# mingdeyu/DGP

Measured on AMD Instinct MI355X. Metric: SI iterations/sec (train) + predict pts/sec, 2-layer DGP n=2000 d=5, higher is better.
Workload: dtype f64; 1 GPU; configs[1]: 2-layer DGP, d=5 in / 1 out, n=2000, Matern-2.5, 5+1 GP nodes, train(ess_burn=10): one step = imputer.sample() + the M-step = one iteration of dgp.train (dgp.py:1364-1412); the same rate over a train(N=100) call is in `sustained`

## Files before the change

### dgp_amd/_lib.py

```python
import ctypes as C
import os

_HERE = os.path.dirname(os.path.abspath(__file__))
LIB_PATH = os.environ.get('DGPAMD_LIB') or os.path.join(_HERE, 'libdgp_amd.so')

OK, NOT_PD, BAD_ARG, HIP_ERROR = 0, 1, 2, 3
SEXP, MATERN25 = 0, 1
MAXD, MAXB = 64, 64
KIND = {'sexp': SEXP, 'matern2.5': MATERN25}

if not os.path.exists(LIB_PATH):
    raise ImportError(
        'dgp_amd: %s not found -- build it with `python -c "import __graft_entry__ as g; g.build()"` '
        '(or `make -C dgp_amd/csrc`).  dgp_amd has no CPU fallback.' % LIB_PATH)

lib = C.CDLL(LIB_PATH)

_p = C.c_void_p
_i = C.c_int
_l = C.c_int64
_d = C.c_double
_z = C.c_size_t

class Node(C.Structure):
# ... 29 lines not shown
    'dgpamd_set_linkgp_direct': (_i, [_p, _i]),
    'dgpamd_set_potrf_mode': (_i, [_p, _i]),
    'dgpamd_debug_trace': (_i, [_p, _p]),
    'dgpamd_debug_tasklog': (_i, [_p, _p, C.c_longlong]),
    'dgpamd_debug_mega_table': (_i, [_p, _l, _i, _i, _p, _l]),
    'dgpamd_prof_enable': (_i, [_p, _i]),
    'dgpamd_prof_event_overhead_us': (_i, [_p, C.POINTER(_d)]),
    'dgpamd_prof_collect': (_i, [_p, C.POINTER(_l), C.POINTER(_d), C.POINTER(_d)]),
    'dgpamd_kmatrix': (_i, [_p, _i, _l, _p, _l, _l, _p, _i, _p, _i, _p, _i, _d, _p, _p, _l, _l, _i, _p, _l, _l, _i, _i]),
    'dgpamd_potrf_workspace': (_z, [_l, _i]),
    'dgpamd_potrf': (_i, [_p, _l, _p, _l, _i, _p, _p, _p]),
    'dgpamd_aug_quad': (_i, [_p, _l, _p, _l, _i, _i, _p]),
    'dgpamd_loglik_finish': (_i, [_p, _l, _p, _l, _i, _p, _d, _p]),
    'dgpamd_loglik': (_i, [_p, _i, _l, _p, _l, _l, _p, _i, _p, _i, _p, _i, _d, _p, _d, _p, _p, _l, _i, _p, _p, _p]),
    'dgpamd_trmv_lower': (_i, [_p, _l, _p, _l, _p, _p, _p, _i]),
    'dgpamd_lik_workspace': (_z, [_i]),
    'dgpamd_lik_loglik': (_i, [_p, _p, _l, _i, _p, _l, _i, _p, _p]),
    'dgpamd_ess_propose': (_i, [_p, _l, _i, _p, _p, _p, _i, _p]),
    'dgpamd_potri': (_i, [_p, _l, _p, _p, _i, _p]),
    'dgpamd_potri_batched': (_i, [_p, _l, _p, _p, _l, _i, _i, _p]),
    'dgpamd_grad_workspace': (_z, [_l, _i]),
    'dgpamd_grad_reduce': (_i, [_p, _i, _l, _p, _l, _p, _i, _p, _i, _p, _i, _d, _p, _i, _p, _p, _p]),
    'dgpamd_ess_update': (_i, [_p, _l, _i, _p, _p, _p, _d, _d, _p, _p, _i, _i, _i, _p, _p, _p, _p, _p, _p]),
    'dgpamd_ess_queue_scratch': (_z, []),
    'dgpamd_ess_queue': (_i, [_p, _l, _i, _p, _p, _i, _p, _p, _i, _p, _p, _p, _i, _i, _i, _i, _i, _p, _p, _p, _p, _p]),
    'dgpamd_ess_queue_vwork': (_z, [_l, _i, _i]),
    'dgpamd_ess_queue_note_info': (_i, [_p, _p, _p, _i]),
    'dgpamd_llik_batch': (_i, [_p, _l, _i, _p, _p, _p, _p, _l, _p, _p, _p, _p, _l]),
    'dgpamd_llik_batch_launch': (_i, [_p, _l, _i, _p, _p, _p, _p, _l, _p, _p, _p, _l]),
    'dgpamd_llik_batch_wait': (_i, [_p, _p]),
# ... 60 lines not shown
```

### dgp_amd/csrc/chol.hip

```cpp
#include "common.hpp"
#include "tile.hpp"
#include "diagfac.hpp"

__device__ __forceinline__ void diag_logdet(DiagShared &sh, int ncol, int k, int b, int bad, double *logdet, int32_t *info) {
    const int tid = threadIdx.x;
    if (tid < 64) {
        const double pv = sh.piv[tid];
        double v = (tid < ncol && pv > 0.0) ? log(pv) : 0.0;
#pragma unroll
        for (int off = 32; off > 0; off >>= 1) v += __shfl_down(v, off, 64);
        if (tid == 0) {
            const double ld0 = k == 0 ? 0.0 : __hip_atomic_load(logdet + b, __ATOMIC_RELAXED, __HIP_MEMORY_SCOPE_AGENT);
            __hip_atomic_store(logdet + b, ld0 + v, __ATOMIC_RELAXED, __HIP_MEMORY_SCOPE_AGENT);
            int inf = k == 0 ? 0 : __hip_atomic_load(info + b, __ATOMIC_RELAXED, __HIP_MEMORY_SCOPE_AGENT);
            if (bad && inf == 0) inf = k * 64 + bad;
            __hip_atomic_store(info + b, inf, __ATOMIC_RELAXED, __HIP_MEMORY_SCOPE_AGENT);
        }
    }
}

enum { G_TRTRI1 = 2, G_TRTRI2 = 3, G_LAUUM = 4 };

struct GemmArgs {
    double *A;
// ... 1153 lines not shown
    const double *z;
    double *out;
    double sscale[DGPAMD_MAXB];
};
__global__ __launch_bounds__(256) void trmv_lower_kernel(TrmvArgs a) {
    const int b = blockIdx.y, wave = threadIdx.x >> 6, lane = threadIdx.x & 63;
    const int64_t i = (int64_t)blockIdx.x * 4 + wave;
    if (i >= a.n) return;
    const double *row = a.L + (int64_t)b * a.stride_a + i * a.ld;
    const double *z = a.z + (int64_t)b * a.n;
    double s = 0.0;
    for (int64_t j = lane; j <= i; j += 64) s = fma(row[j], z[j], s);
#pragma unroll
    for (int off = 32; off > 0; off >>= 1) s += __shfl_down(s, off, 64);
    if (lane == 0) a.out[(int64_t)b * a.n + i] = a.sscale[b] * s;
}

size_t potrf_ws_doubles(int64_t n, int batch) {
    int64_t nbk = padded_dim(n) / 64;
    return (size_t)batch * nbk * 4096 + 2 * DGPAMD_MAXB;
}

static size_t mega_sync_bytes(int64_t nbk, int batch);
static size_t mega_sync_offset(int64_t n, int batch) {
    const size_t b = potrf_ws_doubles(n, batch) * sizeof(double) + 3 * DGPAMD_MAXB * sizeof(int32_t);
    return (b + 127) / 128 * 128;
}
static size_t mega_piv_offset(int64_t n, int batch) {
    return mega_sync_offset(n, batch) + mega_sync_bytes(padded_dim(n) / 64, batch);
}
// ... 498 lines not shown
}

extern "C" int dgpamd_trmv_lower(dgpamd_ctx *ctx, int64_t n, const double *L, int64_t stride_a, const double *scale_h,
                                 const double *z, double *out, int batch) {
    if (!ctx) return DGPAMD_BAD_ARG;
    if (n <= 0 || !L || !z || !out || !scale_h) BAD_ARG(ctx, "null pointer or n <= 0");
    if (batch <= 0 || batch > DGPAMD_MAXB) BAD_ARG(ctx, "need 1 <= batch <= DGPAMD_MAXB");
    TrmvArgs a;
    a.L = L; a.ld = padded_dim(n); a.stride_a = stride_a; a.n = n; a.z = z; a.out = out;
    for (int b = 0; b < batch; ++b) a.sscale[b] = sqrt(scale_h[b]);
    hipLaunchKernelGGL(trmv_lower_kernel, dim3((unsigned)((n + 3) / 4), batch), dim3(256), 0, ctx->stream, a);
    LAUNCH_CHECK(ctx);
    return DGPAMD_OK;
}

static int potri_launches(dgpamd_ctx *ctx, int64_t n, double *A, double *Ainv, int64_t stride_a, int r, int batch,
                          void *work);

extern "C" int dgpamd_potri_batched(dgpamd_ctx *ctx, int64_t n, double *A, double *Ainv, int64_t stride_a, int r,
                                    int batch, void *work) {
    if (!ctx) return DGPAMD_BAD_ARG;
    if (n <= 0 || !A || !Ainv || !work || r < 0) BAD_ARG(ctx, "null pointer or n <= 0");
    if (batch <= 0 || batch > DGPAMD_MAXB) BAD_ARG(ctx, "need 1 <= batch <= DGPAMD_MAXB");
    const int64_t Np = padded_dim(n);
    if (n + r > Np) BAD_ARG(ctx, "too many right-hand sides");
    if (batch > 1 && stride_a < Np * Np) BAD_ARG(ctx, "stride_a < Np*Np");
    const std::array<uint64_t, 10> key = {2, (uint64_t)n, (uint64_t)r, (uint64_t)A, (uint64_t)Ainv, (uint64_t)work,
                                          (uint64_t)batch, (uint64_t)stride_a, 0, 0};
    return graph_run(ctx, key, [&]() { return potri_launches(ctx, n, A, Ainv, stride_a, r, batch, work); });
}
// ... 30 lines not shown
```

### dgp_amd/csrc/train.hip

```cpp
#include "common.hpp"
#include "wave.hpp"

#include <math.h>

struct ProposeArgs {
    const double *F, *NU;
    double *FP;
    int64_t count;
    double th[DGPAMD_MAXB];
};
__global__ __launch_bounds__(256) void ess_propose_kernel(ProposeArgs a) {
    const int b = blockIdx.y;
    const double c = cos(a.th[b]), s = sin(a.th[b]);
    for (int64_t i = (int64_t)blockIdx.x * 256 + threadIdx.x; i < a.count; i += (int64_t)gridDim.x * 256)
        a.FP[(int64_t)b * a.count + i] = a.F[i] * c + a.NU[i] * s;
}

extern "C" int dgpamd_ess_propose(dgpamd_ctx *ctx, int64_t n, int M, const double *F, const double *NU,
                                  const double *theta_h, int batch, double *FP) {
    if (!ctx) return DGPAMD_BAD_ARG;
    if (n <= 0 || M <= 0 || !F || !NU || !theta_h || !FP) BAD_ARG(ctx, "null pointer or empty block");
    if (batch <= 0 || batch > DGPAMD_MAXB) BAD_ARG(ctx, "need 1 <= batch <= DGPAMD_MAXB");
    ProposeArgs a;
    a.F = F; a.NU = NU; a.FP = FP; a.count = n * M;
// ... 641 lines not shown
                HIP_TRY(ctx, hipMemcpyAsync(F, FP + (int64_t)b * n * M, sizeof(double) * n * M, hipMemcpyDeviceToDevice,
                                            ctx->stream));
                return finish(0, llh[b], 0);
            }
        }
        used += nb - 1;
        proposals += nb;
        theta = th[nb - 1]; lo = blo[nb - 1]; hi = bhi[nb - 1];
        pending = true;
    }
}

enum { ES_THETA = 0, ES_LO, ES_HI, ES_PENDING, ES_CURSOR, ES_STATUS, ES_INFO, ES_LL, ES_LOGY, ES_PROPOSALS, ES_BATCHES,
       ES_UPDATES, ES_NWORDS = DGPAMD_ESS_STATE };
struct EssScratch {
    double th[DGPAMD_MAXB], lo[DGPAMD_MAXB], hi[DGPAMD_MAXB], cs[DGPAMD_MAXB], sn[DGPAMD_MAXB], ll[DGPAMD_MAXB], logdet[DGPAMD_MAXB];
    int32_t info[DGPAMD_MAXB], infomax[DGPAMD_MAXB];
    int32_t nb, done, acc, halt;
    double likpart[DGPAMD_MAXB * 32];
};
#define ESS_TWO_PI 6.283185307179586

__device__ void ess_prepare(double *st, const double *u, int nuni, int B, EssScratch *sc);
__global__ void ess_begin_kernel(double *st, const double *u, const double *logu, int nuni, EssScratch *sc, int upd, int B, int resume) {
    if (threadIdx.x) return;
    if (resume && upd == 0) {
        sc->done = 0;
        sc->halt = 0;
        ess_prepare(st, u, nuni, B, sc);
        return;
    }
    if (upd > 0 && !sc->done && st[ES_STATUS] == 0.0) st[ES_STATUS] = 3.0;
    sc->acc = -1;
    sc->nb = 0;
    if (st[ES_STATUS] != 0.0) { sc->done = 1; sc->halt = 1; return; }
    int cur = (int)st[ES_CURSOR];
    if (cur + 2 > nuni) { st[ES_STATUS] = 4.0; sc->done = 1; sc->halt = 1; return; }
    st[ES_LOGY] = st[ES_LL] + logu[cur];
    const double theta = ESS_TWO_PI * u[cur + 1];
    st[ES_THETA] = theta; st[ES_LO] = theta - ESS_TWO_PI; st[ES_HI] = theta; st[ES_PENDING] = 0.0;
    st[ES_CURSOR] = cur + 2;
    sc->done = 0;
    sc->halt = 0;
    ess_prepare(st, u, nuni, B, sc);
}
__device__ void ess_prepare(double *st, const double *u, int nuni, int B, EssScratch *sc) {
    sc->acc = -1;
    sc->nb = 0;
    if (sc->done) return;
    int cur = (int)st[ES_CURSOR];
    double theta = st[ES_THETA], lo = st[ES_LO], hi = st[ES_HI];
    if (st[ES_PENDING] != 0.0) {
        if (cur >= nuni) { st[ES_STATUS] = 1.0; sc->done = 1; return; }
        if (theta < 0.0) lo = theta; else hi = theta;
        theta = __dadd_rn(lo, __dmul_rn(hi - lo, u[cur++]));
        st[ES_THETA] = theta; st[ES_LO] = lo; st[ES_HI] = hi; st[ES_PENDING] = 0.0; st[ES_CURSOR] = cur;
    }
    int nb = 1;
    sc->th[0] = theta; sc->lo[0] = lo; sc->hi[0] = hi;
    while (nb < B && cur + nb - 1 < nuni) {
        if (theta < 0.0) lo = theta; else hi = theta;
        theta = __dadd_rn(lo, __dmul_rn(hi - lo, u[cur + nb - 1]));
        sc->th[nb] = theta; sc->lo[nb] = lo; sc->hi[nb] = hi;
        ++nb;
    }
    for (int b = nb; b < B; ++b) sc->th[b] = sc->th[nb - 1];
    for (int b = 0; b < B; ++b) { sc->cs[b] = cos(sc->th[b]); sc->sn[b] = sin(sc->th[b]); }
    sc->nb = nb;
}
__global__ void ess_prepare_kernel(double *st, const double *u, int nuni, int B, EssScratch *sc) {
    if (threadIdx.x) return;
    ess_prepare(st, u, nuni, B, sc);
}
__global__ __launch_bounds__(256) void ess_propose_dev_kernel(const double *F, const double *NU, double *FP, int64_t count,
                                                              const EssScratch *sc) {
    if (sc->done) return;
    const int b = blockIdx.y;
    const double c = sc->cs[b], s = sc->sn[b];
    for (int64_t i = (int64_t)blockIdx.x * 256 + threadIdx.x; i < count; i += (int64_t)gridDim.x * 256)
        FP[(int64_t)b * count + i] = F[i] * c + NU[i] * s;
}
__device__ void ess_decide(double *st, EssScratch *sc);
__global__ void ess_node_ll_kernel(const double *A, int64_t ld, int64_t stride_a, int64_t n, double scale, int B, int first,
                                   EssScratch *sc, const double *ld_ws, const int32_t *info_ws, const int32_t *status, double *st) {
    const int b = threadIdx.x;
    if (sc->done) return;
    if (b < B) {
        const double logdet = ld_ws ? __hip_atomic_load(ld_ws + b, __ATOMIC_RELAXED, __HIP_MEMORY_SCOPE_AGENT) : sc->logdet[b];
        const int32_t info = ld_ws ? ((status && __hip_atomic_load(status, __ATOMIC_RELAXED, __HIP_MEMORY_SCOPE_AGENT))
                                          ? -1 : __hip_atomic_load(info_ws + b, __ATOMIC_RELAXED, __HIP_MEMORY_SCOPE_AGENT))
                                   : sc->info[b];
        const double quad = -A[(int64_t)b * stride_a + n * ld + n];
        const double ll = -0.5 * ((double)n * log(scale) + logdet + quad / scale);
        sc->ll[b] = (first ? 0.0 : sc->ll[b]) + ll;
        sc->infomax[b] = first ? info : (sc->infomax[b] ? sc->infomax[b] : info);
    }
    if (st) {
        __threadfence_block();
        __syncthreads();
        if (b == 0) ess_decide(st, sc);
    }
}
__device__ void ess_decide(double *st, EssScratch *sc) {
    if (sc->done) return;
    const int nb = sc->nb;
    int cur = (int)st[ES_CURSOR];
    st[ES_BATCHES] += 1.0;
    for (int b = 0; b < nb; ++b) {
        if (sc->infomax[b] != 0) {
            st[ES_STATUS] = 2.0; st[ES_INFO] = sc->infomax[b]; st[ES_PROPOSALS] += b + 1; sc->done = 1;
            return;
        }
        if (sc->ll[b] > st[ES_LOGY]) {
            st[ES_CURSOR] = cur + b; st[ES_PROPOSALS] += b + 1;
            st[ES_THETA] = sc->th[b]; st[ES_LO] = sc->lo[b]; st[ES_HI] = sc->hi[b]; st[ES_PENDING] = 0.0;
            st[ES_LL] = sc->ll[b]; st[ES_UPDATES] += 1.0;
            sc->acc = b; sc->done = 1;
            return;
        }
    }
    st[ES_CURSOR] = cur + nb - 1; st[ES_PROPOSALS] += nb;
    st[ES_THETA] = sc->th[nb - 1]; st[ES_LO] = sc->lo[nb - 1]; st[ES_HI] = sc->hi[nb - 1]; st[ES_PENDING] = 1.0;
}
__global__ __launch_bounds__(256) void ess_accept_kernel(double *F, const double *FP, int64_t count, const EssScratch *sc) {
    const int acc = sc->acc;
    if (acc < 0) return;
    for (int64_t i = (int64_t)blockIdx.x * 256 + threadIdx.x; i < count; i += (int64_t)gridDim.x * 256)
        F[i] = FP[(int64_t)acc * count + i];
}
__global__ void ess_end_kernel(double *st, EssScratch *sc) {
    if (threadIdx.x) return;
    if (!sc->done && st[ES_STATUS] == 0.0) st[ES_STATUS] = 3.0;
    sc->acc = -1;
}
__global__ void ess_set_ll_kernel(double *st, const EssScratch *sc) {
    if (threadIdx.x) return;
    if (st[ES_STATUS] != 0.0) return;
    if (sc->infomax[0] != 0) { st[ES_STATUS] = 2.0; st[ES_INFO] = sc->infomax[0]; }
    st[ES_LL] = sc->ll[0];
}
__global__ void ess_note_info_kernel(double *st, const int32_t *info, int count) {
    if (threadIdx.x || st[ES_STATUS] != 0.0) return;
    for (int i = 0; i < count; ++i)
// ... 21 lines not shown
        const int64_t src = a.ord[i];
        a.out[(int64_t)b * total + e] = d < a.Dl ? a.X[(int64_t)b * a.stride_x + src * a.M + a.colmap[d]] : a.Xglob[src * a.Dg + (d - a.Dl)];
    }
}
__global__ void ess_vnode_ll_kernel(const double *o, double scale, int B, int first, EssScratch *sc, double *st) {
    const int b = threadIdx.x;
    if (sc->done) return;
    if (b < B) {
        const double ll = -0.5 * (o[2 * b + 1] + o[2 * b] / scale);
        sc->ll[b] = (first ? 0.0 : sc->ll[b]) + ll;
        if (first) sc->infomax[b] = 0;
    }
    if (st) {
        __threadfence_block();
        __syncthreads();
        if (b == 0) ess_decide(st, sc);
    }
}

#define LIK_CHUNKS 32
struct LikArgs {
    const double *X;
    int64_t stride_x;
    int M, kind, ncol, classes;
    int cols[DGPAMD_MAXD];
    const int64_t *rep;
    const double *y;
    int64_t nobs;
    double par;
    double *part;
    const int32_t *pred;
// ... 113 lines not shown
    for (int c = 0; c < LIK_CHUNKS; ++c) s += part[b * LIK_CHUNKS + c];
    out[b] = s;
}
__global__ void ess_liknode_ll_kernel(const double *part, int B, int first, EssScratch *sc, double *st) {
    const int b = threadIdx.x;
    if (sc->done) return;
    if (b < B) {
        double s = 0.0;
        for (int c = 0; c < LIK_CHUNKS; ++c) s += part[b * LIK_CHUNKS + c];
        sc->ll[b] = (first ? 0.0 : sc->ll[b]) + s;
        if (first) sc->infomax[b] = 0;
    }
    if (st) {
        __threadfence_block();
        __syncthreads();
        if (b == 0) ess_decide(st, sc);
    }
}
static int lik_launch(dgpamd_ctx *ctx, const dgpamd_node &nd, int64_t n, int M, const double *X, int64_t stride_x, int B, double *part) {
    if (nd.lik_kind < DGPAMD_LIK_POISSON || nd.lik_kind > DGPAMD_LIK_SOFTMAX) BAD_ARG(ctx, "unknown likelihood");
    if (!nd.y || nd.lik_nobs <= 0 || !nd.colmap || nd.Dl <= 0 || nd.Dl > DGPAMD_MAXD) BAD_ARG(ctx, "incomplete likelihood node");
    static const int need[] = {0, 1, 2, 2, 3, 1, 1, 0, 0};
    if (need[nd.lik_kind] && nd.Dl != need[nd.lik_kind]) BAD_ARG(ctx, "wrong number of latent columns for this likelihood");
    if (nd.lik_kind >= DGPAMD_LIK_ROBUSTMAX && (nd.lik_classes != nd.Dl || nd.Dl < 2)) BAD_ARG(ctx, "one latent column per class");
    if (!nd.lik_rep && nd.lik_nobs != n) BAD_ARG(ctx, "observations and latent rows differ without a replicate map");
    LikArgs a;
    a.X = X; a.stride_x = stride_x; a.M = M; a.kind = nd.lik_kind; a.ncol = nd.Dl; a.classes = nd.lik_classes;
    for (int d = 0; d < nd.Dl; ++d) {
        a.cols[d] = ((const int32_t *)nd.colmap)[d];
        if (a.cols[d] < 0 || a.cols[d] >= M) BAD_ARG(ctx, "latent column out of range");
    }
// ... 8 lines not shown
    int rc = lik_launch(ctx, *node, n, M, X, stride_x, batch, work);
    if (rc) return rc;
    hipLaunchKernelGGL(lik_sum_kernel, dim3(1), dim3(DGPAMD_MAXB), 0, ctx->stream, (const double *)work, batch, out);
    LAUNCH_CHECK(ctx);
    return DGPAMD_OK;
}
extern "C" size_t dgpamd_lik_workspace(int batch) { return (size_t)batch * LIK_CHUNKS * sizeof(double); }

extern "C" size_t dgpamd_ess_queue_scratch(void) { return (sizeof(EssScratch) + 15) / 16 * 16; }
extern "C" size_t dgpamd_ess_queue_vwork(int64_t n, int D, int batch) {
    return ((size_t)batch * n * (D + 2) + 2 * (size_t)batch + 2) * sizeof(double);
}

static int ess_queue_logliks(dgpamd_ctx *ctx, int64_t n, int M, const double *X, int64_t stride_x, int B, const dgpamd_node *nodes,
                             const double *scales_h, int nnodes, double *A, void *work, EssScratch *sc, double *st_decide, void *vwork,
                             int vbatch) {
    const int64_t Np = padded_dim(n);
    double *ws = (double *)work;
    for (int k = 0; k < nnodes; ++k) {
        const dgpamd_node &nd = nodes[k];
        if (nd.lik_kind) {
            int rc = lik_launch(ctx, nd, n, M, X, stride_x, B, sc->likpart);
            if (rc) return rc;
            hipLaunchKernelGGL(ess_liknode_ll_kernel, dim3(1), dim3(DGPAMD_MAXB), 0, ctx->stream, (const double *)sc->likpart, B,
                               k == 0 ? 1 : 0, sc, k == nnodes - 1 ? st_decide : nullptr);
            continue;
        }
        if (!(scales_h[k] > 0.0)) BAD_ARG(ctx, "scale must be positive");
        if (nd.vecch_nn) {
            const int D = nd.Dl + nd.Dg;
            if (!vwork || !nd.vecch_ord || !nd.vecch_nd || !nd.vecch_y || nd.vecch_m < 0) BAD_ARG(ctx, "incomplete Vecchia node");
// ... 21 lines not shown
            hipLaunchKernelGGL(ess_vnode_ll_kernel, dim3(1), dim3(DGPAMD_MAXB), 0, ctx->stream, (const double *)osum, scales_h[k], B,
                               k == 0 ? 1 : 0, sc, k == nnodes - 1 ? st_decide : nullptr);
            continue;
        }
        if (!A || !work) BAD_ARG(ctx, "dense nodes upstairs need A and work");
        KmatArgs a;
        int rc = build_kmat_args(ctx, a, nd.kind, n, X, M, stride_x, (const int32_t *)nd.colmap, nd.Dl, nd.Xglob, nd.Dg, nd.length,
                                 nd.nlen, nd.nugget, nd.W, A, Np, Np * Np, 0, nd.y, n, 0, 1, B);
        if (rc) return rc;
        potrf_sync_area(ctx, n, B, false, ws, &a.zero_ptr, &a.zero_words);
        rc = launch_kmatrix(ctx, a, B);
        if (rc) return rc;
        PotrfPost post;
        rc = run_potrf(ctx, n, A, Np * Np, B, sc->logdet, sc->info, ws, nullptr, nullptr, &post, a.zero_ptr != nullptr);
        if (rc) return rc;
        hipLaunchKernelGGL(ess_node_ll_kernel, dim3(1), dim3(DGPAMD_MAXB), 0, ctx->stream, (const double *)A, Np, Np * Np, n,
                           scales_h[k], B, k == 0 ? 1 : 0, sc, post.pending ? post.ld_ws : nullptr,
                           post.pending ? post.info_ws : nullptr, post.pending ? post.status : nullptr,
                           k == nnodes - 1 ? st_decide : nullptr);
    }
    LAUNCH_CHECK(ctx);
    return DGPAMD_OK;
}

extern "C" int dgpamd_ess_queue(dgpamd_ctx *ctx, int64_t n, int M, double *F, const double *NU, int nupd, const dgpamd_node *nodes,
                                const double *scales_h, int nnodes, double *state, const double *uniforms, const double *log_uniforms,
                                int nuni, int batch_first, int batch_next, int max_batches, int compute_ll0, double *FP, double *A,
                                void *work, void *scratch, void *vwork) {
    if (!ctx) return DGPAMD_BAD_ARG;
    if (n <= 0 || M <= 0 || nupd <= 0 || nnodes <= 0 || !F || !NU || !nodes || !scales_h || !state || !FP || !scratch)
        BAD_ARG(ctx, "null pointer or empty block");
    if (nuni < 0 || (nuni > 0 && (!uniforms || !log_uniforms))) BAD_ARG(ctx, "bad uniform stream");
    if (batch_first <= 0 || batch_first > DGPAMD_MAXB) BAD_ARG(ctx, "need 1 <= batch_first <= DGPAMD_MAXB");
    if (batch_next <= 0 || batch_next > batch_first) batch_next = batch_first;
    if (max_batches < 1) max_batches = 1;
    EssScratch *sc = reinterpret_cast<EssScratch *>(scratch);
    const int64_t count = n * (int64_t)M;
    int64_t blocks = (count + 255) / 256;
    if (blocks > 1024) blocks = 1024;
    int rc;
    HIP_TRY(ctx, hipMemsetAsync(sc, 0, sizeof(EssScratch), ctx->stream));
    const int resume = compute_ll0 == 2 ? 1 : 0;
    if (compute_ll0 == 1) {
        rc = ess_queue_logliks(ctx, n, M, F, 0, 1, nodes, scales_h, nnodes, A, work, sc, nullptr, vwork, batch_first);
        if (rc) return rc;
        hipLaunchKernelGGL(ess_set_ll_kernel, dim3(1), dim3(64), 0, ctx->stream, state, (const EssScratch *)sc);
    }
    for (int u = 0; u < nupd; ++u) {
        const double *NUu = NU + (int64_t)u * count;
        hipLaunchKernelGGL(ess_begin_kernel, dim3(1), dim3(64), 0, ctx->stream, state, uniforms, log_uniforms, nuni, sc, u, batch_first, resume);
        for (int j = 0; j < max_batches; ++j) {
            const int B = j == 0 ? batch_first : batch_next;
            if (j > 0) hipLaunchKernelGGL(ess_prepare_kernel, dim3(1), dim3(64), 0, ctx->stream, state, uniforms, nuni, B, sc);
            hipLaunchKernelGGL(ess_propose_dev_kernel, dim3((unsigned)blocks, B), dim3(256), 0, ctx->stream, (const double *)F, NUu, FP,
                               count, (const EssScratch *)sc);
            ctx->pred = &sc->done;
            rc = ess_queue_logliks(ctx, n, M, FP, count, B, nodes, scales_h, nnodes, A, work, sc, state, vwork, batch_first);
            ctx->pred = nullptr;
            if (rc) return rc;
            hipLaunchKernelGGL(ess_accept_kernel, dim3((unsigned)blocks), dim3(256), 0, ctx->stream, F, (const double *)FP, count,
                               (const EssScratch *)sc);
        }
        if (u == nupd - 1) hipLaunchKernelGGL(ess_end_kernel, dim3(1), dim3(64), 0, ctx->stream, state, sc);
    }
    LAUNCH_CHECK(ctx);
    return DGPAMD_OK;
}

extern "C" int dgpamd_ess_queue_note_info(dgpamd_ctx *ctx, double *state, const int32_t *info, int count) {
    if (!ctx) return DGPAMD_BAD_ARG;
    if (!state || !info || count <= 0) BAD_ARG(ctx, "bad arguments");
    hipLaunchKernelGGL(ess_note_info_kernel, dim3(1), dim3(64), 0, ctx->stream, state, info, count);
    LAUNCH_CHECK(ctx);
    return DGPAMD_OK;
}
```

### dgp_amd/imputation.py

```python
import os
import numpy as np
from numpy.linalg import LinAlgError
from .ops import raise_not_pd
from . import dist as ddist
import torch

from .ops import default_engine
from .kernel_class import TrackedInputs, bind_private, peek

TWO_PI = 2.0 * np.pi
_NO_UPLOAD_AHEAD = bool(__import__('os').environ.get('DGPAMD_NO_UPLOAD_AHEAD'))


class DrawStream:

    def __init__(self, seed=None, z=None, u=None):
        ss = seed if isinstance(seed, np.random.SeedSequence) else np.random.SeedSequence(seed)
        a, b = ss.spawn(2)
        self._gz, self._gu = np.random.default_rng(a), np.random.default_rng(b)
        self._z = None if z is None else [np.asarray(v, dtype=float) for v in z]
        self._ubuf = [] if u is None else [float(v) for v in u]
        self._injected_u = u is not None
        self._zbuf, self._zpos, self._thread = None, 0, None

# ... 666 lines not shown
        if self.draws._z is not None and len(self.all_layer) > 2:
            return None
        e = self.engine
        n, M = self.F[0].shape
        if M > 64:
            return None
        if all_vecch:
            Zd = self._normals_ahead(sweeps, M, n)
            xs = self._vecchia_draws(0, list(range(M)), Zd.permute(1, 0, 2).contiguous())
            if prefetch:
                self.draws.prefetch(sweeps * M * n, engine=e)
            return xs.permute(1, 2, 0).contiguous()
        buf = self._layer_factors(0, list(range(M)))
        Zd = self._normals_ahead(sweeps, M, n)
        scales = [float(nd.scale[0]) for nd in layer]
        out = e.empty(sweeps, M, n)
        for s_ in range(sweeps):
            e.trmv_lower(n, buf, scales, Zd[s_], batch=M, out=out[s_])
        if prefetch:
            self.draws.prefetch(sweeps * M * n, engine=e)
        return out.transpose(1, 2).contiguous()

    def _prior_draw(self, l, cols=None):
        e = self.engine
        layer = self.all_layer[l]
        n, M = self.F[l].shape
        Np = e.padded_dim(n)
        nu = e.zeros(n, M)
        cols = list(range(M)) if cols is None else list(cols)
        dense = [k for k in cols if not layer[k].vecch]
        Z = {k: self.draws.normal(n) for k in cols}
        if dense:
            buf = self._layer_factors(l, dense)
# ... 354 lines not shown
```

### dgp_amd/ops.py

```python
import ctypes as C

import numpy as np
import torch

import os

from . import _lib
from ._lib import lib, KIND

_NO_PINNED_UPLOAD = os.environ.get('DGPAMD_PINNED_UPLOAD') == '0'
_POISON_ALL = os.environ.get('DGPAMD_POISON_LDS') == '2'
_POISON_HBM = os.environ.get('DGPAMD_POISON_HBM') == '1'


class DgpAmdError(RuntimeError):
    pass


class HandoffError(DgpAmdError):
    """The one-launch factorisation gave up waiting for another workgroup (its workgroups were not co-resident: a device
    shared with another process, a debugger, a time-sliced partition).  Not a numerical failure; the per-block-step
    factorisation (Engine.set_potrf_mode(0)) has no such waits -- dgp.train retries the iteration once through it."""


# ... 234 lines not shown
        stride_loc = n * ldloc if Xloc.dim() == 3 else 0
        self._chk(self._enter() or lib.dgpamd_loglik(self.h, KIND[kind], n, _dp(Xloc), ldloc, stride_loc, cmp_, Dl, _dp(Xglob), Dg,
                                    _hp(length), len(length), float(nugget), _dp(W), float(scale), _dp(y), _dp(A),
                                    Np * Np, batch, _dp(ll), _dp(info), _dp(work)))
        return ll, info

    def trmv_lower(self, n, L, scale, z, batch=1, out=None, shared=False):
        Np = self.padded_dim(n)
        sc = _f64(scale)
        if len(sc) == 1 and batch > 1:
            sc = np.repeat(sc, batch)
        if out is None:
            out = self.empty(batch, n)
        self._chk(self._enter() or lib.dgpamd_trmv_lower(self.h, n, _dp(L), 0 if shared else Np * Np, _hp(sc), _dp(z), _dp(out),
                                                          batch))
        return out

    def ess_propose(self, F, NU, thetas, out=None):
        n, M = F.shape
        th = _f64(thetas)
        B = len(th)
        if out is None:
            out = self.empty(B, n, M)
        self._chk(self._enter() or lib.dgpamd_ess_propose(self.h, n, M, _dp(F), _dp(NU), _hp(th), B, _dp(out)))
        return out

    def potri(self, n, A, Ainv, r, work, batch=1):
        Np = self.padded_dim(n)
        self._chk(self._enter() or lib.dgpamd_potri_batched(self.h, n, _dp(A), _dp(Ainv), Np * Np if batch > 1 else 0, r, batch, _dp(work)))
        return Ainv
# ... 850 lines not shown
```

### include/dgp_amd.h

```cpp
#ifndef DGP_AMD_H
#define DGP_AMD_H

#include <stddef.h>
#include <stdint.h>

#ifdef __cplusplus
extern "C" {
#endif

#define DGPAMD_OK 0
#define DGPAMD_NOT_PD 1
#define DGPAMD_BAD_ARG 2
#define DGPAMD_HIP_ERROR 3

#define DGPAMD_SEXP 0
#define DGPAMD_MATERN25 1

#define DGPAMD_MAXD 64
#define DGPAMD_MAXB 64

typedef struct dgpamd_ctx dgpamd_ctx;

int dgpamd_create(int device, void *stream, dgpamd_ctx **out);
int dgpamd_destroy(dgpamd_ctx *ctx);
// ... 38 lines not shown

int dgpamd_loglik_finish(dgpamd_ctx *ctx, int64_t n, const double *A, int64_t stride_a, int batch, const double *logdet,
                         double scale, double *ll);

int dgpamd_gemv(dgpamd_ctx *ctx, int64_t rows, int64_t cols, const double *A, int64_t ld, const double *x, double *out);

int dgpamd_loglik(dgpamd_ctx *ctx, int kind, int64_t n,
                  const double *Xloc, int64_t ldloc, int64_t stride_loc, const int32_t *colmap_h, int Dl,
                  const double *Xglob, int Dg,
                  const double *length_h, int nlen, double nugget, const double *W, double scale,
                  const double *y, double *A, int64_t stride_a, int batch,
                  double *ll, int32_t *info, void *work);

int dgpamd_trmv_lower(dgpamd_ctx *ctx, int64_t n, const double *L, int64_t stride_a, const double *scale_h,
                      const double *z, double *out, int batch);

int dgpamd_ess_propose(dgpamd_ctx *ctx, int64_t n, int M, const double *F, const double *NU,
                       const double *theta_h, int batch, double *FP);

int dgpamd_potri(dgpamd_ctx *ctx, int64_t n, double *A, double *Ainv, int r, void *work);
int dgpamd_potrf_inv(dgpamd_ctx *ctx, int64_t n, double *A, double *T, double *S, int64_t stride_a, int batch,
                     double *logdet, int32_t *info, void *work);

int dgpamd_potri_batched(dgpamd_ctx *ctx, int64_t n, double *A, double *Ainv, int64_t stride_a, int r, int batch,
                         void *work);

typedef struct {
    int kind;
    int Dl, Dg, nlen;
    int nugget_est;
// ... 223 lines not shown
```

Measured before the change: 31.46 SI it/s.

## Fuse ESS begin/prepare into propose kernel and batch multi-column TRMV

The ESS begin and prepare single-thread kernels are folded into the proposal kernel: each workgroup recomputes its theta from a shared-memory window of uniforms, and the last workgroup, picked with an atomic ticket, writes the state back. For single-node layers, the node log-likelihood and accept/reject decision are folded into the accept kernel the same way. Separately, the per-sweep TRMV loop that draws prior samples is replaced by one kernel that handles many right-hand-side columns at once, reusing each loaded row of L. This cuts kernel launches and serial tiny kernels in the ESS loop, at the cost of redundant per-block computation, ticket-based cross-block coordination, and changed FMA rounding in theta updates.

```diff
diff --git a/dgp_amd/_lib.py b/dgp_amd/_lib.py
--- a/dgp_amd/_lib.py
+++ b/dgp_amd/_lib.py
@@ -67,6 +67,7 @@
     'dgpamd_loglik_finish': (_i, [_p, _l, _p, _l, _i, _p, _d, _p]),
     'dgpamd_loglik': (_i, [_p, _i, _l, _p, _l, _l, _p, _i, _p, _i, _p, _i, _d, _p, _d, _p, _p, _l, _i, _p, _p, _p]),
     'dgpamd_trmv_lower': (_i, [_p, _l, _p, _l, _p, _p, _p, _i]),
+    'dgpamd_trmv_lower_multi': (_i, [_p, _l, _p, _l, _p, _p, _p, _i, _i, _l]),
     'dgpamd_lik_workspace': (_z, [_i]),
     'dgpamd_lik_loglik': (_i, [_p, _p, _l, _i, _p, _l, _i, _p, _p]),
     'dgpamd_ess_propose': (_i, [_p, _l, _i, _p, _p, _p, _i, _p]),
diff --git a/dgp_amd/csrc/chol.hip b/dgp_amd/csrc/chol.hip
--- a/dgp_amd/csrc/chol.hip
+++ b/dgp_amd/csrc/chol.hip
@@ -1191,6 +1191,38 @@
 #pragma unroll
     for (int off = 32; off > 0; off >>= 1) s += __shfl_down(s, off, 64);
     if (lane == 0) a.out[(int64_t)b * a.n + i] = a.sscale[b] * s;
+}
+
+#define TRMV_COLS 12
+struct TrmvMultiArgs {
+    TrmvArgs t;
+    int64_t col_stride;
+    int ncols;
+};
+__global__ __launch_bounds__(256) void trmv_lower_multi_kernel(TrmvMultiArgs a) {
+    const int b = blockIdx.y, wave = threadIdx.x >> 6, lane = threadIdx.x & 63;
+    const int64_t i = (int64_t)blockIdx.x * 4 + wave;
+    if (i >= a.t.n) return;
+    const double *row = a.t.L + (int64_t)b * a.t.stride_a + i * a.t.ld;
+    for (int c0 = 0; c0 < a.ncols; c0 += TRMV_COLS) {
+        const int nc = a.ncols - c0 < TRMV_COLS ? a.ncols - c0 : TRMV_COLS;
+        const double *z = a.t.z + (int64_t)c0 * a.col_stride + (int64_t)b * a.t.n;
+        double s[TRMV_COLS];
+#pragma unroll
+        for (int c = 0; c < TRMV_COLS; ++c) s[c] = 0.0;
+        for (int64_t j = lane; j <= i; j += 64) {
+            const double l = row[j];
+#pragma unroll
+            for (int c = 0; c < TRMV_COLS; ++c)
+                if (c < nc) s[c] = fma(l, z[(int64_t)c * a.col_stride + j], s[c]);
+        }
+#pragma unroll
+        for (int c = 0; c < TRMV_COLS; ++c) {
+#pragma unroll
+            for (int off = 32; off > 0; off >>= 1) s[c] += __shfl_down(s[c], off, 64);
+            if (lane == 0 && c < nc) a.t.out[(int64_t)(c0 + c) * a.col_stride + (int64_t)b * a.t.n + i] = a.t.sscale[b] * s[c];
+        }
+    }
 }
 
 size_t potrf_ws_doubles(int64_t n, int batch) {
@@ -1719,6 +1751,22 @@
     return DGPAMD_OK;
 }
 
+extern "C" int dgpamd_trmv_lower_multi(dgpamd_ctx *ctx, int64_t n, const double *L, int64_t stride_a, const double *scale_h,
+                                       const double *z, double *out, int batch, int ncols, int64_t col_stride) {
+    if (!ctx) return DGPAMD_BAD_ARG;
+    if (n <= 0 || !L || !z || !out || !scale_h) BAD_ARG(ctx, "null pointer or n <= 0");
+    if (batch <= 0 || batch > DGPAMD_MAXB) BAD_ARG(ctx, "need 1 <= batch <= DGPAMD_MAXB");
+    if (ncols <= 0) BAD_ARG(ctx, "need ncols >= 1");
+    if (ncols > 1 && col_stride < (int64_t)batch * n) BAD_ARG(ctx, "col_stride < batch * n");
+    TrmvMultiArgs a;
+    a.t.L = L; a.t.ld = padded_dim(n); a.t.stride_a = stride_a; a.t.n = n; a.t.z = z; a.t.out = out;
+    for (int b = 0; b < batch; ++b) a.t.sscale[b] = sqrt(scale_h[b]);
+    a.col_stride = col_stride; a.ncols = ncols;
+    hipLaunchKernelGGL(trmv_lower_multi_kernel, dim3((unsigned)((n + 3) / 4), batch), dim3(256), 0, ctx->stream, a);
+    LAUNCH_CHECK(ctx);
+    return DGPAMD_OK;
+}
+
 static int potri_launches(dgpamd_ctx *ctx, int64_t n, double *A, double *Ainv, int64_t stride_a, int r, int batch,
                           void *work);
 
diff --git a/dgp_amd/csrc/train.hip b/dgp_amd/csrc/train.hip
--- a/dgp_amd/csrc/train.hip
+++ b/dgp_amd/csrc/train.hip
@@ -679,119 +679,228 @@
 enum { ES_THETA = 0, ES_LO, ES_HI, ES_PENDING, ES_CURSOR, ES_STATUS, ES_INFO, ES_LL, ES_LOGY, ES_PROPOSALS, ES_BATCHES,
        ES_UPDATES, ES_NWORDS = DGPAMD_ESS_STATE };
 struct EssScratch {
-    double th[DGPAMD_MAXB], lo[DGPAMD_MAXB], hi[DGPAMD_MAXB], cs[DGPAMD_MAXB], sn[DGPAMD_MAXB], ll[DGPAMD_MAXB], logdet[DGPAMD_MAXB];
+    double th[DGPAMD_MAXB], lo[DGPAMD_MAXB], hi[DGPAMD_MAXB], spare[2 * DGPAMD_MAXB], ll[DGPAMD_MAXB], logdet[DGPAMD_MAXB];
     int32_t info[DGPAMD_MAXB], infomax[DGPAMD_MAXB];
     int32_t nb, done, acc, halt;
+    int32_t ticket, fill_;
     double likpart[DGPAMD_MAXB * 32];
 };
 #define ESS_TWO_PI 6.283185307179586
 
-__device__ void ess_prepare(double *st, const double *u, int nuni, int B, EssScratch *sc);
-__global__ void ess_begin_kernel(double *st, const double *u, const double *logu, int nuni, EssScratch *sc, int upd, int B, int resume) {
-    if (threadIdx.x) return;
-    if (resume && upd == 0) {
-        sc->done = 0;
-        sc->halt = 0;
-        ess_prepare(st, u, nuni, B, sc);
-        return;
-    }
-    if (upd > 0 && !sc->done && st[ES_STATUS] == 0.0) st[ES_STATUS] = 3.0;
-    sc->acc = -1;
-    sc->nb = 0;
-    if (st[ES_STATUS] != 0.0) { sc->done = 1; sc->halt = 1; return; }
-    int cur = (int)st[ES_CURSOR];
-    if (cur + 2 > nuni) { st[ES_STATUS] = 4.0; sc->done = 1; sc->halt = 1; return; }
-    st[ES_LOGY] = st[ES_LL] + logu[cur];
-    const double theta = ESS_TWO_PI * u[cur + 1];
-    st[ES_THETA] = theta; st[ES_LO] = theta - ESS_TWO_PI; st[ES_HI] = theta; st[ES_PENDING] = 0.0;
-    st[ES_CURSOR] = cur + 2;
-    sc->done = 0;
-    sc->halt = 0;
-    ess_prepare(st, u, nuni, B, sc);
-}
-__device__ void ess_prepare(double *st, const double *u, int nuni, int B, EssScratch *sc) {
-    sc->acc = -1;
-    sc->nb = 0;
-    if (sc->done) return;
-    int cur = (int)st[ES_CURSOR];
-    double theta = st[ES_THETA], lo = st[ES_LO], hi = st[ES_HI];
-    if (st[ES_PENDING] != 0.0) {
-        if (cur >= nuni) { st[ES_STATUS] = 1.0; sc->done = 1; return; }
+__device__ __forceinline__ double ess_rounded(double x) {
+    asm volatile("" : "+v"(x));
+    return x;
+}
+#define ESS_UWIN (DGPAMD_MAXB + 4)
+struct EssUniforms {
+    const double *win;
+    int base;
+    __device__ __forceinline__ double operator()(int i) const { return win[i - base]; }
+};
+struct EssOpened {
+    int done;
+    double theta;
+};
+template <bool W>
+__device__ __forceinline__ EssOpened ess_open(double *st, const EssUniforms &u, const double *logu, int nuni, EssScratch *sc, int upd, int B,
+                                              int resume, int sel) {
+    int done = sc->done;
+    double status = st[ES_STATUS], curd = st[ES_CURSOR], theta = st[ES_THETA], lo = st[ES_LO], hi = st[ES_HI], pending = st[ES_PENDING];
+    EssOpened r;
+    r.theta = theta;
+    if (upd >= 0) {
+        if (resume && upd == 0) {
+            done = 0;
+            if (W) { sc->done = 0; sc->halt = 0; }
+        } else {
+            if (upd > 0 && !done && status == 0.0) {
+                status = 3.0;
+                if (W) st[ES_STATUS] = 3.0;
+            }
+            if (W) { sc->acc = -1; sc->nb = 0; }
+            const int cur = (int)curd;
+            if (status != 0.0 || cur + 2 > nuni) {
+                if (W) {
+                    if (status == 0.0) st[ES_STATUS] = 4.0;
+                    sc->done = 1;
+                    sc->halt = 1;
+                }
+                r.done = 1;
+                return r;
+            }
+            const double u1 = u(cur + 1);
+            theta = ess_rounded(ESS_TWO_PI * u1);
+            lo = fma(ESS_TWO_PI, u1, -ESS_TWO_PI);
+            hi = theta;
+            pending = 0.0;
+            curd = cur + 2;
+            done = 0;
+            if (W) {
+                st[ES_LOGY] = st[ES_LL] + logu[cur];
+                st[ES_THETA] = theta; st[ES_LO] = lo; st[ES_HI] = hi; st[ES_PENDING] = 0.0;
+                st[ES_CURSOR] = curd;
+                sc->done = 0;
+                sc->halt = 0;
+            }
+        }
+    }
+    if (W) { sc->acc = -1; sc->nb = 0; }
+    r.done = done;
+    if (done) return r;
+    int cur = (int)curd;
+    if (pending != 0.0) {
+        if (cur >= nuni) {
+            if (W) { st[ES_STATUS] = 1.0; sc->done = 1; }
+            r.done = 1;
+            return r;
+        }
         if (theta < 0.0) lo = theta; else hi = theta;
-        theta = __dadd_rn(lo, __dmul_rn(hi - lo, u[cur++]));
-        st[ES_THETA] = theta; st[ES_LO] = lo; st[ES_HI] = hi; st[ES_PENDING] = 0.0; st[ES_CURSOR] = cur;
+        theta = fma(hi - lo, u(cur), lo);
+        ++cur;
+        if (W) { st[ES_THETA] = theta; st[ES_LO] = lo; st[ES_HI] = hi; st[ES_PENDING] = 0.0; st[ES_CURSOR] = cur; }
     }
     int nb = 1;
-    sc->th[0] = theta; sc->lo[0] = lo; sc->hi[0] = hi;
+    if (W) { sc->th[0] = theta; sc->lo[0] = lo; sc->hi[0] = hi; }
+    r.theta = theta;
     while (nb < B && cur + nb - 1 < nuni) {
         if (theta < 0.0) lo = theta; else hi = theta;
-        theta = __dadd_rn(lo, __dmul_rn(hi - lo, u[cur + nb - 1]));
-        sc->th[nb] = theta; sc->lo[nb] = lo; sc->hi[nb] = hi;
+        theta = fma(hi - lo, u(cur + nb - 1), lo);
+        if (W) { sc->th[nb] = theta; sc->lo[nb] = lo; sc->hi[nb] = hi; }
+        if (nb <= sel) r.theta = theta;
         ++nb;
     }
-    for (int b = nb; b < B; ++b) sc->th[b] = sc->th[nb - 1];
-    for (int b = 0; b < B; ++b) { sc->cs[b] = cos(sc->th[b]); sc->sn[b] = sin(sc->th[b]); }
-    sc->nb = nb;
-}
-__global__ void ess_prepare_kernel(double *st, const double *u, int nuni, int B, EssScratch *sc) {
-    if (threadIdx.x) return;
-    ess_prepare(st, u, nuni, B, sc);
-}
-__global__ __launch_bounds__(256) void ess_propose_dev_kernel(const double *F, const double *NU, double *FP, int64_t count,
-                                                              const EssScratch *sc) {
-    if (sc->done) return;
-    const int b = blockIdx.y;
-    const double c = sc->cs[b], s = sc->sn[b];
-    for (int64_t i = (int64_t)blockIdx.x * 256 + threadIdx.x; i < count; i += (int64_t)gridDim.x * 256)
-        FP[(int64_t)b * count + i] = F[i] * c + NU[i] * s;
-}
-__device__ void ess_decide(double *st, EssScratch *sc);
-__global__ void ess_node_ll_kernel(const double *A, int64_t ld, int64_t stride_a, int64_t n, double scale, int B, int first,
-                                   EssScratch *sc, const double *ld_ws, const int32_t *info_ws, const int32_t *status, double *st) {
+    if (W) {
+        for (int b = nb; b < B; ++b) sc->th[b] = theta;
+        sc->nb = nb;
+    }
+    return r;
+}
+__device__ __forceinline__ bool ess_last_workgroup(int32_t *ticket, int *flag_lds) {
+    __syncthreads();
+    if (threadIdx.x == 0) {
+        const int total = (int)(gridDim.x * gridDim.y);
+        const int t = __hip_atomic_fetch_add(ticket, 1, __ATOMIC_RELAXED, __HIP_MEMORY_SCOPE_AGENT);
+        if (t == total - 1) __hip_atomic_store(ticket, 0, __ATOMIC_RELAXED, __HIP_MEMORY_SCOPE_AGENT);
+        *flag_lds = t == total - 1;
+    }
+    __syncthreads();
+    return *flag_lds != 0;
+}
+__global__ __launch_bounds__(256) void ess_propose_dev_kernel(const double *F, const double *NU, double *FP, int64_t count, double *st,
+                                                              const double *u, const double *logu, int nuni, EssScratch *sc, int upd,
+                                                              int B, int resume) {
+    __shared__ double uwin[ESS_UWIN];
+    __shared__ double cs[2];
+    __shared__ int flag[2];
+    const int tid = threadIdx.x, b = blockIdx.y;
+    if (upd < 0 && sc->done) {
+        if (tid == 0 && blockIdx.x == 0 && b == 0) { sc->acc = -1; sc->nb = 0; }
+        return;
+    }
+    EssUniforms uu;
+    uu.win = uwin;
+    uu.base = (int)st[ES_CURSOR];
+    if (tid < ESS_UWIN) uwin[tid] = (uu.base + tid >= 0 && uu.base + tid < nuni) ? u[uu.base + tid] : 0.0;
+    __syncthreads();
+    if (tid == 0) {
+        const EssOpened o = ess_open<false>(st, uu, logu, nuni, sc, upd, B, resume, b);
+        flag[0] = o.done;
+        if (!o.done) { cs[0] = cos(o.theta); cs[1] = sin(o.theta); }
+    }
+    __syncthreads();
+    if (!flag[0]) {
+        const double c = cs[0], s = cs[1];
+        for (int64_t i = (int64_t)blockIdx.x * 256 + tid; i < count; i += (int64_t)gridDim.x * 256)
+            FP[(int64_t)b * count + i] = F[i] * c + NU[i] * s;
+    }
+    if (!ess_last_workgroup(&sc->ticket, &flag[1])) return;
+    if (tid == 0) (void)ess_open<true>(st, uu, logu, nuni, sc, upd, B, resume, 0);
+}
+struct EssNodeLl {
+    const double *A;
+    int64_t ld, stride_a, n;
+    double scale;
+    int B, first;
+    const double *ld_ws;
+    const int32_t *info_ws, *status;
+};
+__device__ __forceinline__ void ess_node_ll(const EssNodeLl &a, const EssScratch *sc, int b, double &ll_out, int32_t &info_out) {
+    const double logdet = a.ld_ws ? __hip_atomic_load(a.ld_ws + b, __ATOMIC_RELAXED, __HIP_MEMORY_SCOPE_AGENT) : sc->logdet[b];
+    const int32_t info = a.ld_ws ? ((a.status && __hip_atomic_load(a.status, __ATOMIC_RELAXED, __HIP_MEMORY_SCOPE_AGENT))
+                                        ? -1 : __hip_atomic_load(a.info_ws + b, __ATOMIC_RELAXED, __HIP_MEMORY_SCOPE_AGENT))
+                                 : sc->info[b];
+    const double quad = -a.A[(int64_t)b * a.stride_a + a.n * a.ld + a.n];
+    const double ll = ess_rounded(-0.5 * (fma((double)a.n, log(a.scale), logdet) + quad / a.scale));
+    const double prev = a.first ? 0.0 : sc->ll[b];
+    ll_out = prev + ll;
+    info_out = a.first ? info : (sc->infomax[b] ? sc->infomax[b] : info);
+}
+template <bool W>
+__device__ __forceinline__ int ess_decide(double *st, EssScratch *sc, const double *ll, const int32_t *infomax) {
+    if (sc->done) return -1;
+    const int nb = sc->nb;
+    int cur = (int)st[ES_CURSOR];
+    if (W) st[ES_BATCHES] += 1.0;
+    for (int b = 0; b < nb; ++b) {
+        if (infomax[b] != 0) {
+            if (W) { st[ES_STATUS] = 2.0; st[ES_INFO] = infomax[b]; st[ES_PROPOSALS] += b + 1; sc->done = 1; }
+            return -1;
+        }
+        if (ll[b] > st[ES_LOGY]) {
+            if (W) {
+                st[ES_CURSOR] = cur + b; st[ES_PROPOSALS] += b + 1;
+                st[ES_THETA] = sc->th[b]; st[ES_LO] = sc->lo[b]; st[ES_HI] = sc->hi[b]; st[ES_PENDING] = 0.0;
+                st[ES_LL] = ll[b]; st[ES_UPDATES] += 1.0;
+                sc->acc = b; sc->done = 1;
+            }
+            return b;
+        }
+    }
+    if (W) {
+        st[ES_CURSOR] = cur + nb - 1; st[ES_PROPOSALS] += nb;
+        st[ES_THETA] = sc->th[nb - 1]; st[ES_LO] = sc->lo[nb - 1]; st[ES_HI] = sc->hi[nb - 1]; st[ES_PENDING] = 1.0;
+    }
+    return -1;
+}
+__global__ void ess_node_ll_kernel(EssNodeLl a, EssScratch *sc, double *st) {
     const int b = threadIdx.x;
     if (sc->done) return;
-    if (b < B) {
-        const double logdet = ld_ws ? __hip_atomic_load(ld_ws + b, __ATOMIC_RELAXED, __HIP_MEMORY_SCOPE_AGENT) : sc->logdet[b];
-        const int32_t info = ld_ws ? ((status && __hip_atomic_load(status, __ATOMIC_RELAXED, __HIP_MEMORY_SCOPE_AGENT))
-                                          ? -1 : __hip_atomic_load(info_ws + b, __ATOMIC_RELAXED, __HIP_MEMORY_SCOPE_AGENT))
-                                   : sc->info[b];
-        const double quad = -A[(int64_t)b * stride_a + n * ld + n];
-        const double ll = -0.5 * ((double)n * log(scale) + logdet + quad / scale);
-        sc->ll[b] = (first ? 0.0 : sc->ll[b]) + ll;
-        sc->infomax[b] = first ? info : (sc->infomax[b] ? sc->infomax[b] : info);
+    if (b < a.B) {
+        double ll;
+        int32_t info;
+        ess_node_ll(a, sc, b, ll, info);
+        sc->ll[b] = ll;
+        sc->infomax[b] = info;
     }
     if (st) {
         __threadfence_block();
         __syncthreads();
-        if (b == 0) ess_decide(st, sc);
-    }
-}
-__device__ void ess_decide(double *st, EssScratch *sc) {
-    if (sc->done) return;
-    const int nb = sc->nb;
-    int cur = (int)st[ES_CURSOR];
-    st[ES_BATCHES] += 1.0;
-    for (int b = 0; b < nb; ++b) {
-        if (sc->infomax[b] != 0) {
-            st[ES_STATUS] = 2.0; st[ES_INFO] = sc->infomax[b]; st[ES_PROPOSALS] += b + 1; sc->done = 1;
-            return;
-        }
-        if (sc->ll[b] > st[ES_LOGY]) {
-            st[ES_CURSOR] = cur + b; st[ES_PROPOSALS] += b + 1;
-            st[ES_THETA] = sc->th[b]; st[ES_LO] = sc->lo[b]; st[ES_HI] = sc->hi[b]; st[ES_PENDING] = 0.0;
-            st[ES_LL] = sc->ll[b]; st[ES_UPDATES] += 1.0;
-            sc->acc = b; sc->done = 1;
-            return;
-        }
-    }
-    st[ES_CURSOR] = cur + nb - 1; st[ES_PROPOSALS] += nb;
-    st[ES_THETA] = sc->th[nb - 1]; st[ES_LO] = sc->lo[nb - 1]; st[ES_HI] = sc->hi[nb - 1]; st[ES_PENDING] = 1.0;
-}
-__global__ __launch_bounds__(256) void ess_accept_kernel(double *F, const double *FP, int64_t count, const EssScratch *sc) {
-    const int acc = sc->acc;
-    if (acc < 0) return;
-    for (int64_t i = (int64_t)blockIdx.x * 256 + threadIdx.x; i < count; i += (int64_t)gridDim.x * 256)
-        F[i] = FP[(int64_t)acc * count + i];
+        if (b == 0) (void)ess_decide<true>(st, sc, sc->ll, sc->infomax);
+    }
+}
+__global__ __launch_bounds__(256) void ess_accept_kernel(double *F, const double *FP, int64_t count, EssScratch *sc, EssNodeLl a, double *st) {
+    __shared__ double ll[DGPAMD_MAXB];
+    __shared__ int32_t infomax[DGPAMD_MAXB];
+    __shared__ int flag[2];
+    const int tid = threadIdx.x;
+    int acc;
+    if (a.A) {
+        if (sc->done) return;
+        if (tid < a.B) ess_node_ll(a, sc, tid, ll[tid], infomax[tid]);
+        __syncthreads();
+        if (tid == 0) flag[0] = ess_decide<false>(st, sc, ll, infomax);
+        __syncthreads();
+        acc = flag[0];
+    } else
+        acc = sc->acc;
+    if (acc >= 0)
+        for (int64_t i = (int64_t)blockIdx.x * 256 + tid; i < count; i += (int64_t)gridDim.x * 256)
+            F[i] = FP[(int64_t)acc * count + i];
+    if (!a.A) return;
+    if (!ess_last_workgroup(&sc->ticket, &flag[1])) return;
+    if (tid < a.B) { sc->ll[tid] = ll[tid]; sc->infomax[tid] = infomax[tid]; }
+    __syncthreads();
+    if (tid == 0) (void)ess_decide<true>(st, sc, ll, infomax);
 }
 __global__ void ess_end_kernel(double *st, EssScratch *sc) {
     if (threadIdx.x) return;
@@ -843,7 +952,7 @@
     if (st) {
         __threadfence_block();
         __syncthreads();
-        if (b == 0) ess_decide(st, sc);
+        if (b == 0) (void)ess_decide<true>(st, sc, sc->ll, sc->infomax);
     }
 }
 
@@ -987,7 +1096,7 @@
     if (st) {
         __threadfence_block();
         __syncthreads();
-        if (b == 0) ess_decide(st, sc);
+        if (b == 0) (void)ess_decide<true>(st, sc, sc->ll, sc->infomax);
     }
 }
 static int lik_launch(dgpamd_ctx *ctx, const dgpamd_node &nd, int64_t n, int M, const double *X, int64_t stride_x, int B, double *part) {
@@ -1026,7 +1135,7 @@
 
 static int ess_queue_logliks(dgpamd_ctx *ctx, int64_t n, int M, const double *X, int64_t stride_x, int B, const dgpamd_node *nodes,
                              const double *scales_h, int nnodes, double *A, void *work, EssScratch *sc, double *st_decide, void *vwork,
-                             int vbatch) {
+                             int vbatch, EssNodeLl *fold) {
     const int64_t Np = padded_dim(n);
     double *ws = (double *)work;
     for (int k = 0; k < nnodes; ++k) {
@@ -1078,10 +1187,16 @@
         PotrfPost post;
         rc = run_potrf(ctx, n, A, Np * Np, B, sc->logdet, sc->info, ws, nullptr, nullptr, &post, a.zero_ptr != nullptr);
         if (rc) return rc;
-        hipLaunchKernelGGL(ess_node_ll_kernel, dim3(1), dim3(DGPAMD_MAXB), 0, ctx->stream, (const double *)A, Np, Np * Np, n,
-                           scales_h[k], B, k == 0 ? 1 : 0, sc, post.pending ? post.ld_ws : nullptr,
-                           post.pending ? post.info_ws : nullptr, post.pending ? post.status : nullptr,
-                           k == nnodes - 1 ? st_decide : nullptr);
+        EssNodeLl ea;
+        ea.A = A; ea.ld = Np; ea.stride_a = Np * Np; ea.n = n; ea.scale = scales_h[k]; ea.B = B; ea.first = k == 0 ? 1 : 0;
+        ea.ld_ws = post.pending ? post.ld_ws : nullptr;
+        ea.info_ws = post.pending ? post.info_ws : nullptr;
+        ea.status = post.pending ? post.status : nullptr;
+        if (fold && st_decide && nnodes == 1)
+            *fold = ea;
+        else
+            hipLaunchKernelGGL(ess_node_ll_kernel, dim3(1), dim3(DGPAMD_MAXB), 0, ctx->stream, ea, sc,
+                               k == nnodes - 1 ? st_decide : nullptr);
     }
     LAUNCH_CHECK(ctx);
     return DGPAMD_OK;
@@ -1106,24 +1221,24 @@
     HIP_TRY(ctx, hipMemsetAsync(sc, 0, sizeof(EssScratch), ctx->stream));
     const int resume = compute_ll0 == 2 ? 1 : 0;
     if (compute_ll0 == 1) {
-        rc = ess_queue_logliks(ctx, n, M, F, 0, 1, nodes, scales_h, nnodes, A, work, sc, nullptr, vwork, batch_first);
+        rc = ess_queue_logliks(ctx, n, M, F, 0, 1, nodes, scales_h, nnodes, A, work, sc, nullptr, vwork, batch_first, nullptr);
         if (rc) return rc;
         hipLaunchKernelGGL(ess_set_ll_kernel, dim3(1), dim3(64), 0, ctx->stream, state, (const EssScratch *)sc);
     }
     for (int u = 0; u < nupd; ++u) {
         const double *NUu = NU + (int64_t)u * count;
-        hipLaunchKernelGGL(ess_begin_kernel, dim3(1), dim3(64), 0, ctx->stream, state, uniforms, log_uniforms, nuni, sc, u, batch_first, resume);
         for (int j = 0; j < max_batches; ++j) {
             const int B = j == 0 ? batch_first : batch_next;
-            if (j > 0) hipLaunchKernelGGL(ess_prepare_kernel, dim3(1), dim3(64), 0, ctx->stream, state, uniforms, nuni, B, sc);
             hipLaunchKernelGGL(ess_propose_dev_kernel, dim3((unsigned)blocks, B), dim3(256), 0, ctx->stream, (const double *)F, NUu, FP,
-                               count, (const EssScratch *)sc);
+                               count, state, uniforms, log_uniforms, nuni, sc, j == 0 ? u : -1, B, resume);
             ctx->pred = &sc->done;
-            rc = ess_queue_logliks(ctx, n, M, FP, count, B, nodes, scales_h, nnodes, A, work, sc, state, vwork, batch_first);
+            EssNodeLl fold;
+            memset(&fold, 0, sizeof(fold));
+            rc = ess_queue_logliks(ctx, n, M, FP, count, B, nodes, scales_h, nnodes, A, work, sc, state, vwork, batch_first, &fold);
             ctx->pred = nullptr;
             if (rc) return rc;
-            hipLaunchKernelGGL(ess_accept_kernel, dim3((unsigned)blocks), dim3(256), 0, ctx->stream, F, (const double *)FP, count,
-                               (const EssScratch *)sc);
+            hipLaunchKernelGGL(ess_accept_kernel, dim3((unsigned)blocks), dim3(256), 0, ctx->stream, F, (const double *)FP, count, sc,
+                               fold, state);
         }
         if (u == nupd - 1) hipLaunchKernelGGL(ess_end_kernel, dim3(1), dim3(64), 0, ctx->stream, state, sc);
     }
diff --git a/dgp_amd/imputation.py b/dgp_amd/imputation.py
--- a/dgp_amd/imputation.py
+++ b/dgp_amd/imputation.py
@@ -704,9 +704,7 @@
         buf = self._layer_factors(0, list(range(M)))
         Zd = self._normals_ahead(sweeps, M, n)
         scales = [float(nd.scale[0]) for nd in layer]
-        out = e.empty(sweeps, M, n)
-        for s_ in range(sweeps):
-            e.trmv_lower(n, buf, scales, Zd[s_], batch=M, out=out[s_])
+        out = e.trmv_lower_multi(n, buf, scales, Zd.contiguous())
         if prefetch:
             self.draws.prefetch(sweeps * M * n, engine=e)
         return out.transpose(1, 2).contiguous()
diff --git a/dgp_amd/ops.py b/dgp_amd/ops.py
--- a/dgp_amd/ops.py
+++ b/dgp_amd/ops.py
@@ -272,6 +272,20 @@
             out = self.empty(batch, n)
         self._chk(self._enter() or lib.dgpamd_trmv_lower(self.h, n, _dp(L), 0 if shared else Np * Np, _hp(sc), _dp(z), _dp(out),
                                                           batch))
+        return out
+
+    def trmv_lower_multi(self, n, L, scale, z, out=None):
+        ncols, batch = int(z.shape[0]), int(z.shape[1])
+        Np = self.padded_dim(n)
+        sc = _f64(scale)
+        if len(sc) == 1 and batch > 1:
+            sc = np.repeat(sc, batch)
+        assert z.is_contiguous() and z.shape[2] == n and len(sc) == batch
+        if out is None:
+            out = self.empty(ncols, batch, n)
+        assert out.is_contiguous() and out.shape == z.shape
+        self._chk(self._enter() or lib.dgpamd_trmv_lower_multi(self.h, n, _dp(L), Np * Np, _hp(sc), _dp(z), _dp(out), batch,
+                                                                ncols, batch * n))
         return out
 
     def ess_propose(self, F, NU, thetas, out=None):
diff --git a/include/dgp_amd.h b/include/dgp_amd.h
--- a/include/dgp_amd.h
+++ b/include/dgp_amd.h
@@ -76,6 +76,8 @@
 
 int dgpamd_trmv_lower(dgpamd_ctx *ctx, int64_t n, const double *L, int64_t stride_a, const double *scale_h,
                       const double *z, double *out, int batch);
+int dgpamd_trmv_lower_multi(dgpamd_ctx *ctx, int64_t n, const double *L, int64_t stride_a, const double *scale_h,
+                            const double *z, double *out, int batch, int ncols, int64_t col_stride);
 
 int dgpamd_ess_propose(dgpamd_ctx *ctx, int64_t n, int M, const double *F, const double *NU,
                        const double *theta_h, int batch, double *FP);
```

Result: no change. 31.58 SI it/s, median of 2 (+0.4%).
